# apache/horaedb

Hardware: NVIDIA H100
Metric: scanned rows/s (higher is better)
Workload: dtype f64

## Files before the change

horaedb_b200/csrc/fused_scan.cu:

```cuda
#include "fused_scan.h"

#include "block_scan.h"

#include <algorithm>
#include <chrono>
#include <cstdlib>

namespace horae {
namespace fused {

namespace {

constexpr int MAXC = 8;
constexpr int kWarpsPerCta = 8;

struct alignas(16) FRec {
  uint32_t item, local;
  uint64_t gkey;
  int64_t bucket;
  uint64_t count;
  double sum, mn, mx;
  uint64_t _pad;
};

struct VSeg { const uint8_t* base1; uint32_t n0, _pad; };

enum : uint32_t { K_RAW64 = 0, K_U32 = 1, K_I32 = 2, K_F32 = 3 };
inline uint32_t kind_of(uint32_t t) {
  return (t == T_U64 || t == T_I64 || t == T_F64) ? K_RAW64 : (t == T_F32 ? K_F32 : ((t == T_I8 || t == T_I16 || t == T_I32) ? K_I32 : K_U32));
}
constexpr uint64_t kI32KeyLo = (1ull << 63) - (1ull << 31), kI32KeyHi = (1ull << 63) + (1ull << 31) - 1;
constexpr int kHot = 4;

struct FParams {
  const SstDev* ssts;
  const RgSel* sel;
  const uint32_t* d_nsel;
  const uint8_t* const* bases;
  uint32_t split;
  uint32_t pcol[MAX_PREDS], pcls[MAX_PREDS];
  uint32_t pbloom[MAX_PREDS];
  uint64_t phash[MAX_PREDS];
  int nslots;
  uint32_t col[MAXC], kind[MAXC], cls[MAXC];
  int npk;
  int has_group, has_ts, value_slot, global_mode;
  int hot_slot[kHot];
  uint64_t hot_flip[kHot], hot_lo[kHot], hot_span[kHot];
  int hot_haspred[kHot];
  int npred;
  int pslot[MAX_PREDS];
  uint32_t pop[MAX_PREDS];
  uint64_t plit[MAX_PREDS];
  int64_t window_ms;
  const uint8_t* scratch;
  uint64_t scratch_stride;
  int region[MAXC];
  int value_stored;
  VSeg* vseg;
  FRec* rec;
  uint32_t rec_cap;
  uint32_t* item_cnt;
  unsigned int* work;
  unsigned long long* counters;
  int* err;
};

__device__ __forceinline__ uint64_t ld_bytes8(const uint8_t* p) {
  uintptr_t a = reinterpret_cast<uintptr_t>(p);
  uint32_t sh = uint32_t(a & 7) * 8;
  const uint64_t* q = reinterpret_cast<const uint64_t*>(a & ~uintptr_t(7));
  uint64_t lo = __ldg(q), hi = __ldg(q + 1);
  return (lo >> sh) | ((hi << 1) << (63 - sh));
}
__device__ __forceinline__ uint32_t ld32u(const uint8_t* p) { return uint32_t(ld_bytes8(p)); }

__device__ __forceinline__ uint64_t widen_kind(uint64_t raw, uint32_t kind) {
  uint32_t r = uint32_t(raw);
  uint64_t v = raw;
  v = kind == K_U32 ? uint64_t(r) : v;
  v = kind == K_I32 ? uint64_t(int64_t(int32_t(r))) : v;
  v = kind == K_F32 ? uint64_t(__double_as_longlong(double(__uint_as_float(r)))) : v;
  return v;
}
__device__ __forceinline__ uint64_t load_kind(const uint8_t* base, uint32_t kind, uint32_t row) {
  return widen_kind(ld_bytes8(base + size_t(row) * (kind == K_RAW64 ? 8u : 4u)), kind);
}

__device__ __forceinline__ uint32_t literal_header(const uint8_t* p, uint32_t* len) {
  const uint32_t t = __ldg(p);
  uint32_t l = t >> 2, hdr = 1;
  if (l >= 60) {
    const uint32_t nb = l - 59;
    l = 0;
    for (uint32_t i = 0; i < nb; i++) l |= uint32_t(__ldg(p + 1 + i)) << (8 * i);
    hdr = 1 + nb;
  }
  *len = l + 1;
  return hdr;
}

__device__ __forceinline__ const uint8_t* slot_base_chase(const FParams& P, uint32_t si, int s) {
  RgSel rs = P.sel[si];
  SstDev sst = P.ssts[rs.sst];
  ChunkDev cd = sst.chunks[size_t(rs.rg) * sst.ncols + P.col[s]];
  PageDev pg = sst.pages[cd.first_page];
  const uint8_t* body = sst.bytes + pg.payload_off;
  const bool is_value = P.value_stored && s == P.value_slot;
  if (cd.codec == 1) {
    if (is_value && cd.stored) {
      const uint8_t* p = body;
      while (__ldg(p) & 0x80) p++;
      p++;
      uint32_t len0 = 0, len1 = 0;
      const uint32_t h0 = literal_header(p, &len0);
      const uint8_t* lit0 = p + h0;
      const uint32_t prefix = cd.optional ? 4 + ld32u(lit0) : 0;
      const uint32_t w = P.kind[s] == K_RAW64 ? 8u : 4u;
      VSeg v;
      v.n0 = (len0 - prefix) / w;
      v._pad = 0;
      v.base1 = lit0 + prefix;
      if (lit0 + len0 < body + pg.comp_size) v.base1 = lit0 + len0 + literal_header(lit0 + len0, &len1);
      P.vseg[si] = v;
      return lit0 + prefix;
    }
    body = P.scratch + rs.scratch_off + uint64_t(P.region[s]) * P.scratch_stride;
  }
  if (cd.optional) {
    uint32_t lv = ld32u(body);
    if (lv > pg.uncomp_size) { lv = 0; atomicExch(P.err, 202); }
    body += 4 + lv;
  }
  if (is_value) { VSeg v; v.base1 = body; v.n0 = rs.num_rows; v._pad = 0; P.vseg[si] = v; }
  return body;
}
__device__ __forceinline__ const uint8_t* slot_base(const FParams& P, uint32_t si, int s) { return P.bases[size_t(si) * MAXC + s]; }
__device__ __noinline__ uint64_t fetch_val(const FParams& P, uint32_t si, int s, uint32_t row) {
  return load_kind(slot_base(P, si, s), P.kind[s], row);
}

struct Bucket { int64_t start, lo, hi; };
__device__ __noinline__ Bucket bucket_range(int64_t ts, int64_t w) {
  constexpr int64_t kMin = INT64_MIN, kMax = INT64_MAX;
  const int64_t r = w - 1;
  Bucket b;
  b.start = ts / w * w;
  if (b.start > 0) { b.lo = b.start; b.hi = b.start > kMax - r ? kMax : b.start + r; }
  else if (b.start < 0) { b.lo = b.start < kMin + r ? kMin : b.start - r; b.hi = b.start; }
  else { b.lo = -r; b.hi = r; }
  return b;
}

__device__ __noinline__ bool later_alive_dup(const FParams& P, uint32_t si, uint32_t row) {
  uint64_t pk[MAX_PK];
  for (int k = 0; k < P.npk; k++) pk[k] = fetch_val(P, si, k, row);
  uint32_t nrows = P.sel[si].num_rows;
  uint32_t r = row + 1;
  for (;;) {
    if (r >= nrows) {
      si++;
      if (si >= *P.d_nsel) return false;
      nrows = P.sel[si].num_rows;
      r = 0;
      if (nrows == 0) continue;
    }
    for (int k = 0; k < P.npk; k++)
      if (fetch_val(P, si, k, r) != pk[k]) return false;
    bool ok = true;
    for (int p = 0; p < P.npred && ok; p++) ok = op_holds(cmp_widened(fetch_val(P, si, P.pslot[p], r), P.plit[p], P.cls[P.pslot[p]]), P.pop[p]);
    if (ok) return true;
    r++;
  }
}

__device__ __forceinline__ uint64_t shfl64(uint64_t v, int src) {
  uint32_t lo = __shfl_sync(0xffffffffu, uint32_t(v), src);
  uint32_t hi = __shfl_sync(0xffffffffu, uint32_t(v >> 32), src);
  return (uint64_t(hi) << 32) | lo;
}
__device__ __forceinline__ double shfl_xor_d(double v, int m) {
  uint64_t b = uint64_t(__double_as_longlong(v));
  uint32_t lo = __shfl_xor_sync(0xffffffffu, uint32_t(b), m);
  uint32_t hi = __shfl_xor_sync(0xffffffffu, uint32_t(b >> 32), m);
  return __longlong_as_double((long long)((uint64_t(hi) << 32) | lo));
}

struct Acc {
  bool open;
  uint64_t g;
  int64_t bstart, blo, bhi;
  uint64_t cnt;
  double sum, mn, mx;
};

__device__ __noinline__ void emit(const FParams& P, const Acc& a, uint32_t item, uint32_t local, uint32_t* slots) {
  if (slots[0] == slots[1]) { slots[0] = atomicAdd(&P.work[1], 32u); slots[1] = slots[0] + 32u; }
  unsigned int slot = slots[0]++;
  if (slot < P.rec_cap) {
    FRec r;
    r.item = item; r.local = local; r.gkey = a.g; r.bucket = a.bstart; r.count = a.cnt; r.sum = a.sum; r.mn = a.mn; r.mx = a.mx; r._pad = 0;
    P.rec[slot] = r;
  } else atomicExch(P.err, 201);
}

struct FileDev {
  const RgCol* rgcol;
  const uint32_t* rg_rows;
  uint32_t rg_base, nrg, ncols, _pad;
  const uint8_t* bytes;
};

__global__ void __launch_bounds__(256) slot_bases_kernel(const __grid_constant__ FParams P, const uint8_t** __restrict__ bases, int only_slot) {
  const uint32_t idx = blockIdx.x * blockDim.x + threadIdx.x;
  const uint32_t si = idx / MAXC;
  const int s = int(idx % MAXC);
  if (si >= *P.d_nsel || s >= P.nslots || (only_slot >= 0 && s != only_slot)) return;
  bases[idx] = slot_base_chase(P, si, s);
}

template <bool W4>
__global__ void __launch_bounds__(256) gate_sel_kernel(const __grid_constant__ FParams P, RgSel* __restrict__ sel, int gate_slot, uint64_t flip,
                                                       uint64_t lo, uint64_t span, uint8_t* __restrict__ flags) {
  __shared__ uint32_t s_last;
  const uint32_t nsel = *P.d_nsel;
  for (uint32_t si = blockIdx.x; si < nsel; si += gridDim.x) {
    const uint8_t* base = P.bases[size_t(si) * MAXC + gate_slot];
    const uint32_t nrows = sel[si].num_rows;
    if (threadIdx.x == 0) s_last = 0;
    __syncthreads();
    uint32_t last = 0;
    const bool aligned = (reinterpret_cast<uintptr_t>(base) & 7) == 0;
    if (W4 && aligned) {
      const uint2* b2 = reinterpret_cast<const uint2*>(base);
      const uint32_t npair = nrows >> 1;
#pragma unroll 4
      for (uint32_t i = threadIdx.x; i < npair; i += 256) {
        const uint2 v = __ldg(b2 + i);
        if ((v.x ^ uint32_t(flip)) - uint32_t(lo) <= uint32_t(span)) last = 2 * i + 1;
        if ((v.y ^ uint32_t(flip)) - uint32_t(lo) <= uint32_t(span)) last = 2 * i + 2;
      }
      if ((nrows & 1) && threadIdx.x == 0 && (ld32u(base + size_t(nrows - 1) * 4) ^ uint32_t(flip)) - uint32_t(lo) <= uint32_t(span)) last = nrows;
    } else {
#pragma unroll 4
      for (uint32_t i = threadIdx.x; i < nrows; i += 256) {
        bool pass;
        if (W4) pass = (ld32u(base + size_t(i) * 4) ^ uint32_t(flip)) - uint32_t(lo) <= uint32_t(span);
        else pass = (ld_bytes8(base + size_t(i) * 8) ^ flip) - lo <= span;
        if (pass) last = i + 1;
      }
    }
    for (int d = 16; d > 0; d >>= 1) { const uint32_t o = __shfl_down_sync(0xffffffffu, last, d); last = o > last ? o : last; }
    if ((threadIdx.x & 31) == 0 && last) atomicMax(&s_last, last);
    __syncthreads();
    if (threadIdx.x == 0) {
      const uint32_t l = s_last;
      flags[si] = l ? 1 : 0;
      sel[si].out_row = l ? (l + 1 < nrows ? l + 1 : nrows) : 0;
    }
    __syncthreads();
  }
}

__global__ void __launch_bounds__(1024) compact_sel_kernel(const RgSel* __restrict__ in, const uint8_t* __restrict__ flags, uint32_t* d_nsel,
                                                           RgSel* __restrict__ out, uint32_t* __restrict__ lpt) {
  __shared__ uint32_t s_w[1024 / 32 + 1];
  __shared__ uint32_t s_bin[1024];
  __shared__ uint32_t s_max;
  const uint32_t n = *d_nsel;
  const uint32_t per = (n + 1023u) / 1024u;
  const uint32_t lo = threadIdx.x * per;
  const uint32_t hi = lo + per < n ? lo + per : n;
  uint32_t cnt = 0;
  for (uint32_t i = lo; i < hi; i++) cnt += flags[i] != 0;
  s_bin[threadIdx.x] = 0;
  if (threadIdx.x == 0) s_max = 0;
  uint32_t m;
  uint32_t pos = block_excl_scan<1024>(cnt, &m, s_w);
  uint32_t mx = 0;
  for (uint32_t i = lo; i < hi; i++)
    if (flags[i]) { out[pos++] = in[i]; mx = in[i].out_row > mx ? in[i].out_row : mx; }
  if (lpt) {
    if (mx) atomicMax(&s_max, mx);
    __syncthreads();
    int shift = 0;
    while ((s_max >> shift) > 1023u) shift++;
    const uint32_t per2 = (m + 1023u) / 1024u;
    const uint32_t lo2 = threadIdx.x * per2, hi2 = lo2 + per2 < m ? lo2 + per2 : m;
    for (uint32_t i = lo2; i < hi2; i++) atomicAdd(&s_bin[1023u - (out[i].out_row >> shift)], 1u);
    __syncthreads();
    uint32_t nbin;
    const uint32_t start = block_excl_scan<1024>(s_bin[threadIdx.x], &nbin, s_w);
    s_bin[threadIdx.x] = start;
    __syncthreads();
    for (uint32_t i = lo2; i < hi2; i++) lpt[atomicAdd(&s_bin[1023u - (out[i].out_row >> shift)], 1u)] = i;
  }
  __syncthreads();
  if (threadIdx.x == 0) *d_nsel = m;
}

__global__ void __launch_bounds__(256) prune_rgs_kernel(const __grid_constant__ FParams P, const FileDev* __restrict__ files, int nfiles,
                                                        uint32_t total_rgs, int prune, uint32_t* __restrict__ keep_rows) {
  const uint32_t idx = blockIdx.x * blockDim.x + threadIdx.x;
  if (idx >= total_rgs) return;
  uint32_t f = 0;
  while (f + 1 < uint32_t(nfiles) && idx >= files[f + 1].rg_base) f++;
  const FileDev fd = files[f];
  const uint32_t rg = idx - fd.rg_base;
  const uint32_t rows = fd.rg_rows[rg];
  uint32_t keep = rows > 0;
  if (keep && prune) {
    const RgCol* rc = fd.rgcol + size_t(rg) * fd.ncols;
    for (int p = 0; p < P.npred && keep; p++) {
      const RgCol c = rc[P.pcol[p]];
      if (c.null_all) { keep = 0; break; }
      if (c.has_minmax && !minmax_may_match(c.mn, c.mx, P.plit[p], P.pop[p], P.pcls[p])) keep = 0;
      else if ((prune & 2) && P.pbloom[p] && c.bloom_blocks && !bloom::may_contain(fd.bytes + c.bloom_off, c.bloom_blocks, P.phash[p])) keep = 0;
    }
  }
  keep_rows[idx] = keep ? rows : 0;
}

__global__ void __launch_bounds__(1024) select_rgs_kernel(const FileDev* __restrict__ files, int nfiles, uint32_t total_rgs,
                                                          const uint32_t* keep_rows, RgSel* __restrict__ sel, uint32_t* d_nsel,
                                                          unsigned long long* counters, uint32_t smem_words, uint64_t scratch_per_rg) {
  extern __shared__ uint32_t s_keep[];
  __shared__ uint32_t s_w[1024 / 32 + 1];
  if (smem_words) {
    for (uint32_t i = threadIdx.x; i < total_rgs; i += 1024) s_keep[i] = keep_rows[i];
    __syncthreads();
    keep_rows = s_keep;
  }
  const uint32_t per = (total_rgs + 1023u) / 1024u;
  const uint32_t lo = threadIdx.x * per;
  const uint32_t hi = lo + per < total_rgs ? lo + per : total_rgs;
  uint32_t cnt = 0;
  unsigned long long rows_sel = 0;
  for (uint32_t i = lo; i < hi; i++) { const uint32_t r = keep_rows[i]; cnt += r > 0; rows_sel += r; }
  uint32_t nsel;
  uint32_t pos = block_excl_scan<1024>(cnt, &nsel, s_w);
  if (cnt) {
// ... 143 lines not shown
                                        int64_t ts, double v, double* s_vals, uint32_t* slots, int lane) {
  const double kInf = __longlong_as_double(0x7ff0000000000000LL);
  const bool has_val = P.value_slot >= 0;
  bool ext = keep && acc.open && (!P.has_group || g == acc.g) && (!HAS_TS || (ts >= acc.blo && ts <= acc.bhi));
  if (__ballot_sync(0xffffffffu, ext) == keep_mask) {
    acc.cnt += __popc(keep_mask);
    if (has_val) {
      const bool num = keep && v == v;
      double mn = num ? v : kInf, mx = num ? v : -kInf;
#pragma unroll
      for (int m = 1; m < 32; m <<= 1) {
        const double a = shfl_xor_d(mn, m), b = shfl_xor_d(mx, m);
        const bool later = (lane & m) != 0;
        mn = (later ? a <= mn : a < mn) ? a : mn;
        mx = (later ? b >= mx : b > mx) ? b : mx;
      }
      acc.mn = mn < acc.mn ? mn : acc.mn;
      acc.mx = mx > acc.mx ? mx : acc.mx;
      acc.sum = seq_sum_slice(acc.sum, keep_mask, keep, v, s_vals, lane);
    }
    return;
  }
  uint64_t vb = uint64_t(__double_as_longlong(v));
  while (keep_mask) {
    int l = __ffs(keep_mask) - 1;
    keep_mask &= keep_mask - 1;
    uint64_t kg = P.has_group ? shfl64(g, l) : 0;
    int64_t kt = HAS_TS ? int64_t(shfl64(uint64_t(ts), l)) : 0;
    if (!acc.open || kg != acc.g || (HAS_TS && (kt < acc.blo || kt > acc.bhi))) {
      if (acc.open) { if (lane == 0) emit(P, acc, item, local, slots); local++; }
      acc.open = true; acc.g = kg; acc.cnt = 0; acc.sum = 0.0; acc.mn = kInf; acc.mx = -kInf;
      if (HAS_TS) { Bucket b = bucket_range(kt, P.window_ms); acc.bstart = b.start; acc.blo = b.lo; acc.bhi = b.hi; }
      else { acc.bstart = 0; acc.blo = 0; acc.bhi = 0; }
    }
    acc.cnt++;
    if (has_val) {
      double x = __longlong_as_double((long long)shfl64(vb, l));
      acc.sum += x;
      if (acc.cnt == 1 || x < acc.mn) acc.mn = x;
      if (acc.cnt == 1 || x > acc.mx) acc.mx = x;
    }
  }
}

__device__ __forceinline__ double to_double_kind(uint64_t raw, uint32_t kind, uint32_t cls) {
  uint64_t wv = widen_kind(raw, kind);
  return cls == C_FLOAT ? __longlong_as_double((long long)wv) : (cls == C_SIGNED ? double(int64_t(wv)) : double(wv));
}

__device__ __forceinline__ uint64_t ld8(const uint8_t* q, uint32_t sh, uint32_t i) {
  const uint64_t* p = reinterpret_cast<const uint64_t*>(q) + i;
  uint64_t lo = __ldg(p), hi = __ldg(p + 1);
  uint32_t w0 = uint32_t(lo), w1 = uint32_t(lo >> 32), w2 = uint32_t(hi), w3 = uint32_t(hi >> 32);
  const bool up = (sh & 32u) != 0;
  const uint32_t s = sh & 31u;
  uint32_t a = up ? w1 : w0, b = up ? w2 : w1, c = up ? w3 : w2;
  return (uint64_t(__funnelshift_r(b, c, s)) << 32) | __funnelshift_r(a, b, s);
}
__device__ __forceinline__ uint32_t ld4(const uint8_t* q, uint32_t sh, uint32_t i) {
  const uint32_t* p = reinterpret_cast<const uint32_t*>(q) + i;
  uint32_t lo = __ldg(p), hi = __ldg(p + 1);
  return __funnelshift_r(lo, hi, sh);
}

struct VCur {
  const uint8_t *q0, *q1;
  uint32_t s0, s1;
  uint32_t split;
};
__device__ __forceinline__ uint64_t ldv(const VCur& V, bool v8, uint32_t i) {
  const bool a = i < V.split;
  const uint8_t* q = a ? V.q0 : V.q1;
  const uint32_t sh = a ? V.s0 : V.s1;
  const uint32_t j = a ? i : i - V.split;
  return v8 ? ld8(q, sh, j) : uint64_t(ld4(q, sh, j));
}

template <int NH>
struct Hot {
  const uint8_t* q[NH];
  uint32_t sh[NH];
  uint64_t flip[NH], lo[NH], span[NH];
  bool haspred[NH];
};

template <int kU, int NH, int X, bool HAS_TS, bool dense>
__device__ __forceinline__ uint32_t process_block(const FParams& P, const Hot<NH>& H, const VCur& V, Acc& acc, uint32_t& local,
                                                  uint32_t& n_alive, uint32_t& n_keep, uint32_t& n_full, uint32_t item, uint32_t csi, uint32_t row,
                                                  uint32_t lim, uint32_t nrows, bool pf, double* s_vals, uint32_t* slots, int lane) {
  uint64_t hv[kU][NH];
  uint64_t vv[kU];
  uint64_t halo[2] = {0, 0};
  const uint32_t last = nrows - 1;
  if (pf) {
    const uint32_t prow = row + 2 * 32 * kU;
#pragma unroll
    for (int h = 0; h < NH; h++) {
      const bool w4 = h >= 2 && ((X >> (h - 2)) & 1);
      const uint32_t per_line = w4 ? 32u : 16u;
      const uint32_t r = prow + uint32_t(lane) * per_line;
      if (uint32_t(lane) <= (32u * kU) / per_line && r < nrows)
        asm volatile("prefetch.global.L2 [%0];" ::"l"(H.q[h] + size_t(r) * (w4 ? 4 : 8)));
    }
  }
  n_full += lim - row < 32u * kU ? lim - row : 32u * kU;
#pragma unroll
  for (int u = 0; u < kU; u++) {
    uint32_t i = row + u * 32 + lane;
    i = i < last ? i : last;
#pragma unroll
    for (int h = 0; h < NH; h++) {
      const bool w4 = h >= 2 && ((X >> (h - 2)) & 1);
      hv[u][h] = w4 ? uint64_t(ld4(H.q[h], H.sh[h], i)) : ld8(H.q[h], H.sh[h], i);
    }
  }
  const bool v8 = P.value_slot >= 0 && P.kind[P.value_slot] == K_RAW64;
  if (dense) {
    uint32_t i = row + kU * 32;
    i = i < last ? i : last;
    halo[0] = ld8(H.q[0], H.sh[0], i);
    halo[1] = ld8(H.q[1], H.sh[1], i);
#pragma unroll
    for (int u = 0; u < kU; u++) {
      uint32_t i2 = row + u * 32 + lane;
      i2 = i2 < last ? i2 : last;
      vv[u] = ldv(V, v8, i2);
    }
  }
  uint32_t kept_in_block = 0;
#pragma unroll
  for (int u = 0; u < kU; u++) {
    const uint32_t i = row + u * 32 + lane;
    bool alive = i < lim;
#pragma unroll
    for (int h = 0; h < NH; h++) {
      const bool w4 = h >= 2 && ((X >> (h - 2)) & 1);
      if (H.haspred[h]) {
        if (w4) alive = alive && ((uint32_t(hv[u][h]) ^ uint32_t(H.flip[h])) - uint32_t(H.lo[h]) <= uint32_t(H.span[h]));
        else alive = alive && ((hv[u][h] ^ H.flip[h]) - H.lo[h] <= H.span[h]);
      }
    }
    const unsigned alive_mask = __ballot_sync(0xffffffffu, alive);
    if (alive_mask == 0) continue;
    uint64_t n0 = shfl64(hv[u][0], (lane + 1) & 31), n1 = shfl64(hv[u][1], (lane + 1) & 31);
    if (u + 1 < kU) {
      uint64_t f0 = shfl64(hv[u + 1 < kU ? u + 1 : u][0], 0), f1 = shfl64(hv[u + 1 < kU ? u + 1 : u][1], 0);
      if (lane == 31) { n0 = f0; n1 = f1; }
    } else {
      if (!dense && (alive_mask >> 31)) {
        uint32_t ih = row + kU * 32;
        ih = ih < last ? ih : last;
        halo[0] = ld8(H.q[0], H.sh[0], ih);
        halo[1] = ld8(H.q[1], H.sh[1], ih);
      }
      if (lane == 31) { n0 = halo[0]; n1 = halo[1]; }
    }
    bool keep = alive;
    if (alive) {
      bool same = true;
      if (i + 1 < nrows) {
        same = n0 == hv[u][0] && n1 == hv[u][1];
        for (int k = 2; k < P.npk && same; k++) same = fetch_val(P, csi, k, i + 1) == fetch_val(P, csi, k, i);
      }
      if (same && (i + 1 < nrows || csi + 1 < *P.d_nsel)) keep = !later_alive_dup(P, csi, i);
    }
    const unsigned keep_mask = __ballot_sync(0xffffffffu, keep);
    n_alive += __popc(alive_mask);
    n_keep += __popc(keep_mask);
    kept_in_block += __popc(keep_mask);
    if (!P.global_mode && keep_mask) {
      double v = 0.0;
      if (P.value_slot >= 0) {
        uint64_t raw = vv[u];
        if (!dense) raw = keep ? ldv(V, v8, i) : 0ull;
        v = to_double_kind(raw, P.kind[P.value_slot], P.cls[P.value_slot]);
      }
      walk_slice<HAS_TS>(P, acc, local, item, keep_mask, keep, hv[u][0], int64_t(hv[u][1]), v, s_vals, slots, lane);
    }
  }
  return kept_in_block;
}

template <int kU, int NH, int X, int kGS>
__device__ __forceinline__ uint32_t gate_sweep(const Hot<NH>& H, uint32_t row, uint32_t lim, uint32_t nrows, int lane) {
  constexpr int G = NH - 1;
  constexpr bool w4 = G >= 2 && ((X >> (G - 2)) & 1);
  {
    constexpr uint32_t per_line = w4 ? 32u : 16u;
    const uint32_t r = row + 2u * 32u * kGS + uint32_t(lane) * per_line;
    if (uint32_t(lane) < (32u * kGS) / per_line + 1 && r < nrows)
      asm volatile("prefetch.global.L2 [%0];" ::"l"(H.q[G] + size_t(r) * (w4 ? 4 : 8)));
  }
  const uint32_t last = nrows - 1;
  uint64_t gv[kGS];
#pragma unroll
  for (int u = 0; u < kGS; u++) {
    uint32_t i = row + u * 32 + lane;
    i = i < last ? i : last;
    gv[u] = w4 ? uint64_t(ld4(H.q[G], H.sh[G], i)) : ld8(H.q[G], H.sh[G], i);
  }
  uint32_t bm = 0;
#pragma unroll
  for (int u = 0; u < kGS; u++) {
    bool pass = w4 ? ((uint32_t(gv[u]) ^ uint32_t(H.flip[G])) - uint32_t(H.lo[G]) <= uint32_t(H.span[G]))
                   : ((gv[u] ^ H.flip[G]) - H.lo[G] <= H.span[G]);
    pass = pass && (row + u * 32 + lane < lim);
    if (__ballot_sync(0xffffffffu, pass)) bm |= 1u << (u / kU);
  }
  return bm;
}

template <int kU, int NH, int X, int kGS>
__device__ __forceinline__ void prefetch_blocks(const Hot<NH>& H, const uint8_t* vq, bool has_val, bool v8, uint32_t bm, uint32_t row,
                                                uint32_t nrows, int lane) {
#pragma unroll
  for (int h = 0; h < NH - 1; h++) {
    const bool w4 = h >= 2 && ((X >> (h - 2)) & 1);
    const uint32_t off = uint32_t(lane) * (w4 ? 32u : 16u);
    uint32_t blk = off / (32u * kU);
    blk = blk < uint32_t(kGS / kU) ? blk : uint32_t(kGS / kU) - 1;
    if (off <= 32u * kGS && ((bm >> blk) & 1u) && row + off < nrows)
      asm volatile("prefetch.global.L2 [%0];" ::"l"(H.q[h] + size_t(row + off) * (w4 ? 4 : 8)));
  }
  if (has_val) {
    const uint32_t off = uint32_t(lane) * (v8 ? 16u : 32u);
    uint32_t blk = off / (32u * kU);
    blk = blk < uint32_t(kGS / kU) ? blk : uint32_t(kGS / kU) - 1;
    if (off <= 32u * kGS && ((bm >> blk) & 1u) && row + off < nrows)
      asm volatile("prefetch.global.L2 [%0];" ::"l"(vq + size_t(row + off) * (v8 ? 8 : 4)));
  }
}

template <int kU, int kMinBlocks, int NH, int X, bool HAS_TS, bool GATED>
__global__ void __launch_bounds__(kWarpsPerCta * 32, kMinBlocks) fused_scan_kernel(const __grid_constant__ FParams P,
                                                                                    const uint64_t* __restrict__ adj) {
  __shared__ double s_vals_all[kWarpsPerCta][32];
  __shared__ uint32_t s_slots[kWarpsPerCta][2];
  const int lane = threadIdx.x & 31, wid = threadIdx.x >> 5;
  double* s_vals = s_vals_all[wid];
  uint32_t* slots = s_slots[wid];
  if (lane == 0) { slots[0] = 0; slots[1] = 0; }
  __syncwarp();
  const uint32_t nsel = *P.d_nsel;
  const uint32_t nitems = nsel * P.split;
  constexpr int kGS = ((NH - 1) >= 2 && ((X >> (NH - 3)) & 1)) ? 16 : 8;
  const double kInf = __longlong_as_double(0x7ff0000000000000LL);
  Hot<NH> H;
#pragma unroll
  for (int h = 0; h < NH; h++) {
    H.flip[h] = P.hot_flip[h]; H.lo[h] = P.hot_lo[h]; H.span[h] = P.hot_span[h]; H.haspred[h] = P.hot_haspred[h] != 0;
    H.q[h] = nullptr; H.sh[h] = 0;
  }
  VCur V;
  V.q0 = nullptr; V.q1 = nullptr; V.s0 = 0; V.s1 = 0; V.split = 0xffffffffu;
  auto set_cursor = [&](uint32_t si) {
#pragma unroll
    for (int h = 0; h < NH; h++) {
      const uintptr_t a = reinterpret_cast<uintptr_t>(slot_base(P, si, P.hot_slot[h]));
      const bool w4 = h >= 2 && ((X >> (h - 2)) & 1);
      const uintptr_t m = w4 ? 3 : 7;
      H.q[h] = reinterpret_cast<const uint8_t*>(a & ~m);
      H.sh[h] = uint32_t(a & m) * 8;
    }
    if (P.value_slot >= 0) {
      const uintptr_t a = reinterpret_cast<uintptr_t>(slot_base(P, si, P.value_slot));
      const uintptr_t m = P.kind[P.value_slot] == K_RAW64 ? 7 : 3;
      V.q0 = reinterpret_cast<const uint8_t*>(a & ~m);
      V.s0 = uint32_t(a & m) * 8;
      if (P.value_stored) {
        const VSeg vg = P.vseg[si];
        const uintptr_t b = reinterpret_cast<uintptr_t>(vg.base1);
        V.q1 = reinterpret_cast<const uint8_t*>(b & ~m);
        V.s1 = uint32_t(b & m) * 8;
        V.split = vg.n0;
      }
    }
  };
  for (;;) {
    uint32_t item = 0;
    if (lane == 0) item = atomicAdd(&P.work[0], 1u);
    item = __shfl_sync(0xffffffffu, item, 0);
    if (item >= nitems) {
      if (lane == 0) for (uint32_t sl = slots[0]; sl < slots[1]; sl++) if (sl < P.rec_cap) P.rec[sl].item = 0xffffffffu;
      return;
    }
    const uint64_t beg = adj[item], end = adj[item + 1];
    uint32_t csi = uint32_t(beg >> 32), row = uint32_t(beg);
    const uint32_t esi = uint32_t(end >> 32), erow = uint32_t(end);
    uint32_t local = 0, n_alive = 0, n_keep = 0, n_full = 0;
    if (beg < end) {
      Acc acc;
      acc.open = false; acc.g = 0; acc.bstart = 0; acc.blo = 0; acc.bhi = 0; acc.cnt = 0; acc.sum = 0.0; acc.mn = kInf; acc.mx = -kInf;
      bool dense = false;
      uint32_t bm = 0, sweep_kept = 0;
      uint32_t nrows = P.sel[csi].num_rows;
      set_cursor(csi);
      for (;;) {
        if (row >= nrows) {
          csi++;
          row = 0;
          if (csi > esi || (csi == esi && erow == 0) || csi >= nsel) break;
          nrows = P.sel[csi].num_rows;
          set_cursor(csi);
        }
        const uint32_t lim = csi == esi ? erow : nrows;
        if (row >= lim) break;
        if (dense) {
          const uint32_t kept = process_block<kU, NH, X, HAS_TS, true>(P, H, V, acc, local, n_alive, n_keep, n_full, item, csi, row, lim, nrows,
                                                                      true, s_vals, slots, lane);
          dense = kept >= 32u * kU / 4;
          row += 32 * kU;
          continue;
        }
        uint32_t brow = row;
        if (GATED) {
          if (bm == 0) {
            bm = gate_sweep<kU, NH, X, kGS>(H, row, lim, nrows, lane);
            sweep_kept = 0;
            if (bm == 0) { row += 32u * kGS; continue; }
            prefetch_blocks<kU, NH, X, kGS>(H, V.q0, P.value_slot >= 0, P.value_slot >= 0 && P.kind[P.value_slot] == K_RAW64, bm, row, nrows, lane);
          }
          brow = row + (__ffs(bm) - 1) * 32u * kU;
          bm &= bm - 1;
        }
        const uint32_t kept = process_block<kU, NH, X, HAS_TS, false>(P, H, V, acc, local, n_alive, n_keep, n_full, item, csi, brow, lim, nrows,
                                                                     !GATED, s_vals, slots, lane);
        if (GATED) {
          sweep_kept += kept;
          if (bm == 0) {
            const uint32_t swept = lim - row < 32u * kGS ? lim - row : 32u * kGS;
            dense = P.value_slot >= 0 && sweep_kept >= swept / 4;
            row += 32u * kGS;
          }
        } else {
          dense = P.value_slot >= 0 && kept >= 32u * kU / 4;
          row += 32 * kU;
        }
      }
// ... 167 lines not shown
      if (nhot == kHot) return NOT_APPLICABLE;
      h = nhot++;
      hot_slot[h] = pslot[i];
    }
    uint64_t key = pred_literal(preds[i], t) ^ order_flip(t);
    switch (preds[i].op) {
      case HG_OP_EQ: klo[h] = std::max(klo[h], key); khi[h] = std::min(khi[h], key); break;
      case HG_OP_LT: if (key == 0) empty_interval = true; else khi[h] = std::min(khi[h], key - 1); break;
      case HG_OP_LE: khi[h] = std::min(khi[h], key); break;
      case HG_OP_GT: if (key == ~0ull) empty_interval = true; else klo[h] = std::max(klo[h], key + 1); break;
      default: klo[h] = std::max(klo[h], key); break;
    }
  }
  for (int h = 0; h < kHot; h++) if (klo[h] > khi[h]) empty_interval = true;
  for (int h = 2; h < nhot; h++) {
    const uint32_t t = schema->types[slots[hot_slot[h]]];
    if (type_width(t) == 8) continue;
    if (type_is_signed(t) ? (khi[h] < kI32KeyLo || klo[h] > kI32KeyHi) : klo[h] > 0xffffffffull) empty_interval = true;
  }
  if (nhot == 4 && type_width(schema->types[slots[hot_slot[2]]]) < type_width(schema->types[slots[hot_slot[3]]])) {
    std::swap(hot_slot[2], hot_slot[3]);
    std::swap(klo[2], klo[3]);
    std::swap(khi[2], khi[3]);
  }

  static const bool trace = getenv("HORAE_TRACE") != nullptr;
  auto now = [] { return std::chrono::steady_clock::now(); };
  auto us = [](std::chrono::steady_clock::time_point a, std::chrono::steady_clock::time_point b) { return std::chrono::duration<double, std::micro>(b - a).count(); };
  auto t0 = now();
  std::vector<SstResident*> files;
  uint64_t rows_in_files = 0;
  for (size_t i = 0; i < n; i++) {
    auto it = e->ssts.find(ssts[i].id);
    if (it == e->ssts.end()) return set_error(HG_ERR_INTERNAL, "sst not resident after load");
    SstResident* f = it->second.get();
    rows_in_files += f->rows_total;
    if (f->rows_total == 0) continue;
    for (uint32_t c : slots)
      if (!f->col_all_single[c] || !f->col_null_none[c] || f->col_any_zstd[c]) return NOT_APPLICABLE;
    if (!global_mode && (!f->col_has_minmax[0] || (has_ts && !f->col_has_minmax[1]))) return NOT_APPLICABLE;
    files.push_back(f);
  }
  if (files.size() > 1) {
    std::vector<Pk0Range> ranges;
    std::vector<size_t> order;
    for (SstResident* f : files) ranges.push_back(f->pk0);
    if (!pk0_disjoint(ranges, schema->types[0], &order)) return NOT_APPLICABLE;
    const std::vector<SstResident*> given = files;
    for (size_t j = 0; j < order.size(); j++) files[j] = given[order[j]];
  }
  uint32_t total_rgs = 0;
  for (SstResident* f : files) total_rgs += uint32_t(f->rg_rows.size());
  out->gtype = has_group ? schema->types[0] : uint32_t(T_U64);
  out->gwidth = has_group ? type_width(out->gtype) : 8;
  if (empty_interval) {
    for (DevBuf* b : {&out->gkey, &out->bucket, &out->count, &out->sum, &out->mn, &out->mx}) CU_TRY(b->alloc(16, e->stream));
    out->G = 0;
    e->stats.rows_in_files = rows_in_files;
    e->stats.path = 1;
    return HG_OK;
  }
  bool slot_snappy[MAXC] = {false};
  uint64_t slot_comp[MAXC] = {0};
  uint64_t scratch_stride = 0;
  bool value_stored = false, value_all_stored = true;
  for (size_t i = 0; i < slots.size(); i++)
    for (SstResident* f : files) {
      const uint32_t c = slots[i];
      if (f->col_any_snappy[c]) { slot_snappy[i] = true; scratch_stride = std::max<uint64_t>(scratch_stride, f->col_max_scratch[c]); }
      slot_comp[i] += f->col_comp_bytes[c];
      if (int(i) == value_slot) {
        if (f->col_snappy_any_stored[c]) value_stored = true;
        if (f->col_any_snappy[c] && !f->col_snappy_all_stored[c]) value_all_stored = false;
      }
    }
  if (value_slot >= 0) {
    if (!slot_snappy[value_slot]) value_stored = false;
    for (int h = 0; h < nhot; h++) if (hot_slot[h] == value_slot) value_stored = false;
    for (int k2 = 0; k2 < int(schema->num_primary_keys); k2++) if (k2 == value_slot) value_stored = false;
  }
  scratch_stride = (scratch_stride + 255) & ~uint64_t(255);
  int region[MAXC];
  int nregions = 0;
  for (size_t i = 0; i < slots.size(); i++) region[i] = (slot_snappy[i] && !(value_stored && value_all_stored && int(i) == value_slot)) ? nregions++ : -1;
  const bool need_snappy = nregions > 0;
  auto t1 = now();

  uint64_t bound = 1;
  if (!global_mode) {
    if (type_is_float(schema->types[0])) return NOT_APPLICABLE;
    bound = 0;
    if (!has_ts) {
      for (SstResident* f : files) bound += f->group_bound;
    } else {
      for (SstResident* f : files) {
        const size_t ncols = size_t(f->meta.ncols);
        for (size_t g = 0; g < f->rg_rows.size(); g++) {
          const RgCol* rc = &f->rgcol[g * ncols];
          const uint64_t rows = f->rg_rows[g];
          uint64_t span = rc[0].mx - rc[0].mn + 1;
          uint64_t per = std::min<uint64_t>((rc[1].mx - rc[1].mn) / uint64_t(agg->window_ms), 1ull << 33) + 2;
          uint64_t gcount = (span == 0 || span > (1ull << 32) || per > (1ull << 32)) ? rows : span * per;
          bound += std::min<uint64_t>(gcount, rows) + 1;
        }
      }
    }
    if (bound > rows_in_files / 32 + 1024) return NOT_APPLICABLE;
  }
  if (bound >= 0xfffffff0ull || rows_in_files >= 0xfffffff0ull) return NOT_APPLICABLE;

  cudaStream_t s = e->stream;
  Launch L = e->L();
  uint32_t split = 1;
  static const int items_per_warp = getenv("HORAE_ITEMS_PER_WARP") ? atoi(getenv("HORAE_ITEMS_PER_WARP")) : 4;
  while (split < 8 && uint64_t(total_rgs) * split < uint64_t(kNumSMs) * 32 * uint64_t(items_per_warp)) split *= 2;
  const uint32_t nitems = total_rgs * split;
  DevBuf d_ssts, d_files, d_sel, d_sel2, d_rec, d_item, d_work, d_adj, d_keep, d_bsum, d_bases, d_vseg, d_gflags, d_scratch, d_lpt;
  CU_TRY(d_work.alloc(256, s));
  CU_TRY(cudaMemsetAsync(d_work.p, 0, 256, s));
  uint8_t* const zblock = static_cast<uint8_t*>(d_work.p);
  unsigned long long* const counters_p = reinterpret_cast<unsigned long long*>(zblock + 64);
  int* const err_p = reinterpret_cast<int*>(zblock + 128);
  const uint64_t rec_cap = bound + uint64_t(kNumSMs) * 8 * kWarpsPerCta * 32;
  CU_TRY(d_rec.alloc(size_t(rec_cap) * sizeof(FRec) + 64, s));
  CU_TRY(d_item.alloc(size_t(nitems + 1) * sizeof(uint32_t) + 64, s));
  CU_TRY(d_adj.alloc(size_t(nitems + 2) * sizeof(uint64_t), s));
  CU_TRY(d_sel.alloc(size_t(total_rgs + 1) * sizeof(RgSel), s));
  CU_TRY(d_keep.alloc(size_t(total_rgs + 1) * sizeof(uint32_t), s));
  CU_TRY(d_bsum.alloc(1024 * sizeof(uint32_t), s));
  CU_TRY(d_bases.alloc(size_t(total_rgs + 1) * MAXC * sizeof(uint8_t*), s));
  if (value_stored) CU_TRY(d_vseg.alloc(size_t(total_rgs + 1) * sizeof(VSeg), s));
  if (need_snappy) {
    CU_TRY(d_sel2.alloc(size_t(total_rgs + 1) * sizeof(RgSel), s));
    CU_TRY(d_gflags.alloc(size_t(total_rgs) + 16, s));
    CU_TRY(d_lpt.alloc(size_t(total_rgs + 1) * sizeof(uint32_t), s));
    CU_TRY(d_scratch.alloc(size_t(total_rgs) * size_t(nregions) * scratch_stride + 256, s));
  }
  if ((uint64_t(nitems) + 1023) / 1024 > 1024) return NOT_APPLICABLE;
  CU_TRY(out->gkey.alloc(size_t(bound) * 8 + 16, s));
  CU_TRY(out->bucket.alloc(size_t(bound) * 8 + 16, s));
  CU_TRY(out->count.alloc(size_t(bound) * 8 + 16, s));
  CU_TRY(out->sum.alloc(size_t(bound) * 8 + 16, s));
  CU_TRY(out->mn.alloc(size_t(bound) * 8 + 16, s));
  CU_TRY(out->mx.alloc(size_t(bound) * 8 + 16, s));
  AggOut ao{out->gkey.p, out->bucket.as<int64_t>(), out->count.as<uint64_t>(), out->sum.as<double>(), out->mn.as<double>(), out->mx.as<double>()};

  auto t2 = now();
  unsigned long long hc[4] = {0, 0, 0, 0};
  int herr = 0;
  uint32_t hw[2] = {0, 0};
  if (total_rgs > 0) {
    std::vector<SstDev> sd(files.size());
    std::vector<FileDev> fdv(files.size());
    uint32_t rgb = 0;
    for (size_t i = 0; i < files.size(); i++) {
      SstResident* f = files[i];
      sd[i] = SstDev{f->d_bytes, f->d_pages, f->d_chunks, uint32_t(f->meta.ncols), uint32_t(f->meta.rgs.size())};
      fdv[i] = FileDev{f->d_rgcol, f->d_rg_rows, rgb, uint32_t(f->rg_rows.size()), uint32_t(f->meta.ncols), 0, f->d_bytes};
      rgb += uint32_t(f->rg_rows.size());
    }
    CU_TRY(d_ssts.alloc(sd.size() * sizeof(SstDev), s));
    CU_TRY(d_files.alloc(fdv.size() * sizeof(FileDev), s));
    size_t stage_off = 0;
    int urc = stage_upload(e, d_ssts.p, sd.data(), sd.size() * sizeof(SstDev), &stage_off);
    if (!urc) urc = stage_upload(e, d_files.p, fdv.data(), fdv.size() * sizeof(FileDev), &stage_off);
    if (urc) return urc;

    FParams P;
    std::memset(&P, 0, sizeof(P));
    P.ssts = d_ssts.as<SstDev>();
    P.sel = d_sel.as<RgSel>();
    P.d_nsel = d_work.as<uint32_t>() + 3;
    P.bases = d_bases.as<const uint8_t*>();
    P.split = split;
    P.nslots = int(slots.size());
    for (size_t i = 0; i < slots.size(); i++) {
      uint32_t t = schema->types[slots[i]];
      P.col[i] = slots[i];
      P.kind[i] = kind_of(t);
      P.cls[i] = cmp_class(t);
    }
    P.npk = int(schema->num_primary_keys);
    P.has_group = has_group;
    P.has_ts = has_ts;
    P.value_slot = value_slot;
    P.global_mode = global_mode;
    int xmask = 0;
    for (int h = 0; h < kHot; h++) {
      const int sl = h < nhot ? hot_slot[h] : 0;
      const uint32_t t = schema->types[slots[sl]];
      const bool w8 = (t == T_U64 || t == T_I64 || t == T_F64);
      P.hot_slot[h] = sl;
      P.hot_haspred[h] = (h < nhot && (klo[h] != 0 || khi[h] != ~0ull)) ? 1 : 0;
      uint64_t lo = klo[h], hi = khi[h];
      if (w8) P.hot_flip[h] = order_flip(t);
      else if (type_is_signed(t)) {
        P.hot_flip[h] = 1ull << 31;
        lo = lo < kI32KeyLo ? 0 : lo - kI32KeyLo;
        hi = hi > kI32KeyHi ? 0xffffffffull : hi - kI32KeyLo;
      } else {
        P.hot_flip[h] = 0;
        hi = std::min<uint64_t>(hi, 0xffffffffull);
      }
      P.hot_lo[h] = lo;
      P.hot_span[h] = hi >= lo ? hi - lo : 0;
      if (h >= 2 && h < nhot && !w8) xmask |= 1 << (h - 2);
    }
    P.npred = int(np);
    for (size_t i = 0; i < np; i++) {
      P.pslot[i] = pslot[i];
      P.pop[i] = preds[i].op;
      P.plit[i] = pred_literal(preds[i], schema->types[preds[i].column]);
      P.pcol[i] = preds[i].column;
      P.pcls[i] = cmp_class(schema->types[preds[i].column]);
      P.pbloom[i] = preds[i].op == HG_OP_EQ && bloom_literal_hash(P.plit[i], schema->types[preds[i].column], &P.phash[i]) ? 1u : 0u;
    }
    P.window_ms = has_ts ? agg->window_ms : 1;
    P.scratch = d_scratch.as<uint8_t>();
    P.scratch_stride = scratch_stride;
    for (int i = 0; i < MAXC; i++) P.region[i] = i < int(slots.size()) ? region[i] : -1;
    P.value_stored = value_stored ? 1 : 0;
    P.vseg = d_vseg.as<VSeg>();
    P.rec = d_rec.as<FRec>();
    P.rec_cap = uint32_t(rec_cap);
    P.item_cnt = d_item.as<uint32_t>();
    P.work = d_work.as<unsigned int>();
    P.counters = counters_p;
    P.err = err_p;

    int ctas = int(std::min<uint64_t>((uint64_t(nitems) + kWarpsPerCta - 1) / kWarpsPerCta, uint64_t(kNumSMs) * 8));
    static const bool env_nogate = getenv("HORAE_NO_GATE") != nullptr;
    const bool gated = !env_nogate && !(e->flags & HG_FLAG_NO_LATE_MATERIALIZATION) && P.hot_haspred[nhot - 1] != 0;
    prune_rgs_kernel<<<(total_rgs + 255) / 256, 256, 0, s>>>(P, d_files.as<FileDev>(), int(files.size()), total_rgs,
                                                             (e->flags & HG_FLAG_NO_PRUNING) ? 0 : ((e->flags & HG_FLAG_NO_BLOOM_FILTER) ? 1 : 3),
                                                             d_keep.as<uint32_t>());
    L.tick();
    {
      CU_TRY(cudaFuncSetAttribute(select_rgs_kernel, cudaFuncAttributeMaxDynamicSharedMemorySize, 200 * 1024));
      const uint32_t smem_words = size_t(total_rgs) * 4 <= 200 * 1024 ? total_rgs : 0;
      select_rgs_kernel<<<1, 1024, size_t(smem_words) * 4, s>>>(d_files.as<FileDev>(), int(files.size()), total_rgs, d_keep.as<uint32_t>(),
                                                                d_sel.as<RgSel>(), d_work.as<uint32_t>() + 3, counters_p, smem_words,
                                                                uint64_t(nregions) * scratch_stride);
    }
    L.tick();
    CU_TRY(cudaEventRecord(e->evd0, s));
    if (need_snappy) {
      auto make_job = [&](const std::vector<int>& job_slots, unsigned int* ticket) {
        k::SnappyJob J;
        std::memset(&J, 0, sizeof(J));
        J.ssts = P.ssts; J.sel = P.sel; J.d_nsel = P.d_nsel; J.nsel = 0; J.ncols = int(job_slots.size());
        std::vector<int> ord(job_slots.size());
        for (size_t i = 0; i < ord.size(); i++) ord[i] = int(i);
        std::stable_sort(ord.begin(), ord.end(), [&](int a, int b) { return slot_comp[job_slots[a]] > slot_comp[job_slots[b]]; });
        for (size_t i = 0; i < job_slots.size(); i++) {
          J.col[i] = slots[job_slots[i]];
          J.region[i] = uint32_t(region[job_slots[i]]);
          J.order[i] = uint8_t(ord[i]);
          J.skip_stored[i] = (value_stored && job_slots[i] == value_slot) ? 1 : 0;
        }
        J.fixed_stride = scratch_stride; J.scratch = d_scratch.as<uint8_t>(); J.ticket = ticket; J.err = err_p;
        return J;
      };
      unsigned int* tickets = reinterpret_cast<unsigned int*>(zblock + 136);
      const int gate_slot = hot_slot[nhot - 1];
      std::vector<int> first, rest;
      for (int i = 0; i < int(slots.size()); i++) {
        if (region[i] < 0) continue;
        if (gated && i == gate_slot) first.push_back(i); else rest.push_back(i);
      }
      if (!first.empty()) {
        k::snappy_pages(L, make_job(first, tickets), total_rgs);
        slot_bases_kernel<<<(total_rgs * MAXC + 255) / 256, 256, 0, s>>>(P, d_bases.as<const uint8_t*>(), gate_slot);
        L.tick();
        const uint32_t gt = schema->types[slots[gate_slot]];
        const bool w4 = !(gt == T_U64 || gt == T_I64 || gt == T_F64);
        if (w4) gate_sel_kernel<true><<<kNumSMs * 8, 256, 0, s>>>(P, d_sel.as<RgSel>(), gate_slot, P.hot_flip[nhot - 1], P.hot_lo[nhot - 1], P.hot_span[nhot - 1], d_gflags.as<uint8_t>());
        else gate_sel_kernel<false><<<kNumSMs * 8, 256, 0, s>>>(P, d_sel.as<RgSel>(), gate_slot, P.hot_flip[nhot - 1], P.hot_lo[nhot - 1], P.hot_span[nhot - 1], d_gflags.as<uint8_t>());
        L.tick();
        compact_sel_kernel<<<1, 1024, 0, s>>>(d_sel.as<RgSel>(), d_gflags.as<uint8_t>(), d_work.as<uint32_t>() + 3, d_sel2.as<RgSel>(), d_lpt.as<uint32_t>());
        L.tick();
        P.sel = d_sel2.as<RgSel>();
      }
      if (!rest.empty()) {
        k::SnappyJob J2 = make_job(rest, tickets + 1);
        if (!first.empty() && !has_ts)
          for (size_t i = 0; i < rest.size(); i++) J2.partial[i] = rest[i] != 0 ? 1 : 0;
        if (!first.empty()) { J2.sel = P.sel; J2.lpt = d_lpt.as<uint32_t>(); }
        k::snappy_pages(L, J2, total_rgs * uint32_t(rest.size()));
      }
    }
    CU_TRY(cudaEventRecord(e->evd1, s));
    slot_bases_kernel<<<(total_rgs * MAXC + 255) / 256, 256, 0, s>>>(P, d_bases.as<const uint8_t*>(), -1);
    L.tick();
    {
      const uint32_t nb = (nitems + 1 + kBoundsPerWarp - 1) / kBoundsPerWarp;
      const int bctas = int((uint64_t(nb) * 32 + 255) / 256);
      if (has_ts) item_bounds_kernel<true><<<bctas, 256, 0, s>>>(P, d_adj.as<uint64_t>());
      else item_bounds_kernel<false><<<bctas, 256, 0, s>>>(P, d_adj.as<uint64_t>());
      L.tick();
    }
    CU_TRY(cudaEventRecord(e->evk0, s));
    launch_fused<2, 4>(nhot, xmask, has_ts, gated, ctas, s, P, d_adj.as<uint64_t>());
    L.tick();
    CU_TRY(cudaEventRecord(e->evk1, s));
    if (global_mode) {
      global_count_kernel<<<1, 1, 0, s>>>(counters_p, ao);
      L.tick();
    } else {
      const uint32_t sblocks = (nitems + 1023) / 1024;
      item_scan_kernel<<<sblocks, 1024, 0, s>>>(d_item.as<uint32_t>(), d_work.as<uint32_t>() + 3, split, d_bsum.as<uint32_t>());
      L.tick();
      scatter_records_kernel<<<kNumSMs * 4, 256, 0, s>>>(d_rec.as<FRec>(), d_work.as<unsigned int>() + 1, d_item.as<uint32_t>(), d_bsum.as<uint32_t>(),
                                                     sblocks, d_work.as<uint32_t>() + 2, out->gwidth, ao, uint32_t(std::min<uint64_t>(bound, 0xffffffffu)), uint32_t(std::min<uint64_t>(rec_cap, 0xffffffffu)), err_p);
      L.tick();
    }
    auto t3 = now();
    {
      if (!e->h_small) CU_TRY(cudaMallocHost(&e->h_small, 256));
      uint8_t* const hb = static_cast<uint8_t*>(e->h_small);
      CU_TRY(cudaMemcpyAsync(hb, zblock, 192, cudaMemcpyDeviceToHost, s));
      CU_TRY(cudaStreamSynchronize(s));
      std::memcpy(hw, hb + 4, sizeof(hw));
      std::memcpy(hc, hb + 64, sizeof(hc));
      std::memcpy(&herr, hb + 128, sizeof(int));
    }
    auto t4 = now();
    if (trace) fprintf(stderr, "[fused] plan %.0f us, bound+alloc %.0f us, upload+launch %.0f us, wait %.0f us (row groups %u, max items %u)\n", us(t0, t1), us(t1, t2), us(t2, t3), us(t3, t4), total_rgs, nitems);
    if (herr >= 201 && herr <= 203) return set_error(HG_ERR_FORMAT, "fused scan: rows contradict their chunk statistics or a page is damaged (device error " + std::to_string(herr) + ")");
    if (herr) return set_error(HG_ERR_INTERNAL, "fused scan: device error " + std::to_string(herr));
    float kms = 0;
    cudaEventElapsedTime(&kms, e->evk0, e->evk1);
    e->stats.kernel_ms = kms;
    if (need_snappy) { cudaEventElapsedTime(&kms, e->evd0, e->evd1); e->stats.decomp_ms = kms; }
  }
  out->G = global_mode ? (hc[1] > 0 ? 1u : 0u) : hw[1];
  e->stats.rows_in_files = rows_in_files;
  e->stats.rows_decoded = hc[2];
  e->stats.rows_materialized = hc[3];
  e->stats.rows_filtered = hc[0];
  e->stats.rows_out = hc[1];
  e->stats.groups_out = out->G;
  e->stats.path = 1;
  return HG_OK;
}

}
}
```

Baseline: 51.01 billion.

## Precompute gate predicate bitmaps per row group and reuse them in fused sweep

New measurement: 52.59 billion (median of 6 runs). 3.1% higher.

```diff
diff --git a/horaedb_b200/csrc/fused_scan.cu b/horaedb_b200/csrc/fused_scan.cu
--- a/horaedb_b200/csrc/fused_scan.cu
+++ b/horaedb_b200/csrc/fused_scan.cu
@@ -57,6 +57,8 @@
   uint64_t scratch_stride;
   int region[MAXC];
   int value_stored;
+  int gate_bits;
+  uint64_t bits_off;
   VSeg* vseg;
   FRec* rec;
   uint32_t rec_cap;
@@ -211,52 +213,67 @@
   const uint8_t* bytes;
 };
 
-__global__ void __launch_bounds__(256) slot_bases_kernel(const __grid_constant__ FParams P, const uint8_t** __restrict__ bases, int only_slot) {
+__global__ void __launch_bounds__(256) slot_bases_kernel(const __grid_constant__ FParams P, const uint8_t** __restrict__ bases) {
   const uint32_t idx = blockIdx.x * blockDim.x + threadIdx.x;
   const uint32_t si = idx / MAXC;
   const int s = int(idx % MAXC);
-  if (si >= *P.d_nsel || s >= P.nslots || (only_slot >= 0 && s != only_slot)) return;
+  if (si >= *P.d_nsel || s >= P.nslots) return;
   bases[idx] = slot_base_chase(P, si, s);
 }
 
 template <bool W4>
-__global__ void __launch_bounds__(256) gate_sel_kernel(const __grid_constant__ FParams P, RgSel* __restrict__ sel, int gate_slot, uint64_t flip,
-                                                       uint64_t lo, uint64_t span, uint8_t* __restrict__ flags) {
+__global__ void __launch_bounds__(256, 8) gate_rg_kernel(const __grid_constant__ FParams P, RgSel* __restrict__ sel, int gate_slot, uint64_t flip,
+                                                      uint64_t lo, uint64_t span, uint8_t* __restrict__ flags) {
+  constexpr int kRows = W4 ? 8 : 4;
   __shared__ uint32_t s_last;
+  __shared__ const uint8_t* s_base[256];
   const uint32_t nsel = *P.d_nsel;
-  for (uint32_t si = blockIdx.x; si < nsel; si += gridDim.x) {
-    const uint8_t* base = P.bases[size_t(si) * MAXC + gate_slot];
-    const uint32_t nrows = sel[si].num_rows;
-    if (threadIdx.x == 0) s_last = 0;
-    __syncthreads();
-    uint32_t last = 0;
-    const bool aligned = (reinterpret_cast<uintptr_t>(base) & 7) == 0;
-    if (W4 && aligned) {
-      const uint2* b2 = reinterpret_cast<const uint2*>(base);
-      const uint32_t npair = nrows >> 1;
-#pragma unroll 4
-      for (uint32_t i = threadIdx.x; i < npair; i += 256) {
-        const uint2 v = __ldg(b2 + i);
-        if ((v.x ^ uint32_t(flip)) - uint32_t(lo) <= uint32_t(span)) last = 2 * i + 1;
-        if ((v.y ^ uint32_t(flip)) - uint32_t(lo) <= uint32_t(span)) last = 2 * i + 2;
-      }
-      if ((nrows & 1) && threadIdx.x == 0 && (ld32u(base + size_t(nrows - 1) * 4) ^ uint32_t(flip)) - uint32_t(lo) <= uint32_t(span)) last = nrows;
-    } else {
-#pragma unroll 4
-      for (uint32_t i = threadIdx.x; i < nrows; i += 256) {
-        bool pass;
-        if (W4) pass = (ld32u(base + size_t(i) * 4) ^ uint32_t(flip)) - uint32_t(lo) <= uint32_t(span);
-        else pass = (ld_bytes8(base + size_t(i) * 8) ^ flip) - lo <= span;
-        if (pass) last = i + 1;
-      }
-    }
-    for (int d = 16; d > 0; d >>= 1) { const uint32_t o = __shfl_down_sync(0xffffffffu, last, d); last = o > last ? o : last; }
-    if ((threadIdx.x & 31) == 0 && last) atomicMax(&s_last, last);
-    __syncthreads();
-    if (threadIdx.x == 0) {
-      const uint32_t l = s_last;
-      flags[si] = l ? 1 : 0;
-      sel[si].out_row = l ? (l + 1 < nrows ? l + 1 : nrows) : 0;
+  const int lane = threadIdx.x & 31;
+  for (uint32_t k0 = 0; blockIdx.x + k0 * gridDim.x < nsel; k0 += 256) {
+    {
+      const uint32_t si = blockIdx.x + (k0 + threadIdx.x) * gridDim.x;
+      if (si < nsel) s_base[threadIdx.x] = slot_base_chase(P, si, gate_slot);
+    }
+    for (uint32_t k = 0; k < 256; k++) {
+      const uint32_t si = blockIdx.x + (k0 + k) * gridDim.x;
+      if (si >= nsel) break;
+      if (threadIdx.x == 0) s_last = 0;
+      __syncthreads();
+      const uint8_t* base = s_base[k];
+      const RgSel rs = sel[si];
+      const uint32_t nrows = rs.num_rows;
+      uint32_t* bits = P.gate_bits ? reinterpret_cast<uint32_t*>(const_cast<uint8_t*>(P.scratch) + rs.scratch_off + P.bits_off) : nullptr;
+      const bool aligned = (reinterpret_cast<uintptr_t>(base) & (W4 ? 3 : 7)) == 0;
+      uint32_t last = 0;
+      const uint32_t nw = (nrows + 31) >> 5;
+      for (uint32_t i0 = 0; i0 < nw * 32; i0 += kRows * 256) {
+        uint64_t v[kRows];
+#pragma unroll
+        for (int u = 0; u < kRows; u++) {
+          const uint32_t i = i0 + u * 256 + threadIdx.x;
+          v[u] = 0;
+          if (i < nrows) {
+            if (W4) v[u] = aligned ? __ldg(reinterpret_cast<const uint32_t*>(base) + i) : ld32u(base + size_t(i) * 4);
+            else v[u] = aligned ? __ldg(reinterpret_cast<const unsigned long long*>(base) + i) : ld_bytes8(base + size_t(i) * 8);
+          }
+        }
+#pragma unroll
+        for (int u = 0; u < kRows; u++) {
+          const uint32_t i = i0 + u * 256 + threadIdx.x;
+          const bool pass = i < nrows && (W4 ? (uint32_t(v[u]) ^ uint32_t(flip)) - uint32_t(lo) <= uint32_t(span) : (v[u] ^ flip) - lo <= span);
+          if (pass) last = i + 1;
+          const uint32_t b = __ballot_sync(0xffffffffu, pass);
+          if (bits && lane == 0 && (i >> 5) < nw) bits[i >> 5] = b;
+        }
+      }
+      for (int d = 16; d > 0; d >>= 1) { const uint32_t o = __shfl_down_sync(0xffffffffu, last, d); last = o > last ? o : last; }
+      if (lane == 0 && last) atomicMax(&s_last, last);
+      __syncthreads();
+      if (threadIdx.x == 0) {
+        const uint32_t l = s_last;
+        flags[si] = l ? 1 : 0;
+        sel[si].out_row = l ? (l + 1 < nrows ? l + 1 : nrows) : 0;
+      }
     }
     __syncthreads();
   }
@@ -566,6 +583,7 @@
   uint32_t sh[NH];
   uint64_t flip[NH], lo[NH], span[NH];
   bool haspred[NH];
+  const uint32_t* gbits;
 };
 
 template <int kU, int NH, int X, bool HAS_TS, bool dense>
@@ -669,6 +687,24 @@
 __device__ __forceinline__ uint32_t gate_sweep(const Hot<NH>& H, uint32_t row, uint32_t lim, uint32_t nrows, int lane) {
   constexpr int G = NH - 1;
   constexpr bool w4 = G >= 2 && ((X >> (G - 2)) & 1);
+  if (H.gbits) {
+    const uint32_t* bw = H.gbits;
+    const uint32_t nw = (nrows + 31) >> 5;
+    uint32_t sb = 0;
+    const uint32_t r = row + uint32_t(lane) * 32u;
+    if (lane < kGS && r < lim) {
+      const uint32_t w = r >> 5;
+      const uint32_t a = __ldg(bw + w), b = w + 1 < nw ? __ldg(bw + w + 1) : 0u;
+      sb = __funnelshift_r(a, b, r & 31);
+      if (lim - r < 32) sb &= (1u << (lim - r)) - 1;
+    }
+    const unsigned m = __ballot_sync(0xffffffffu, sb != 0);
+    uint32_t bm = 0;
+#pragma unroll
+    for (int u = 0; u < kGS; u++)
+      if ((m >> u) & 1u) bm |= 1u << (u / kU);
+    return bm;
+  }
   {
     constexpr uint32_t per_line = w4 ? 32u : 16u;
     const uint32_t r = row + 2u * 32u * kGS + uint32_t(lane) * per_line;
@@ -737,7 +773,9 @@
   }
   VCur V;
   V.q0 = nullptr; V.q1 = nullptr; V.s0 = 0; V.s1 = 0; V.split = 0xffffffffu;
+  H.gbits = nullptr;
   auto set_cursor = [&](uint32_t si) {
+    if (GATED && P.gate_bits) H.gbits = reinterpret_cast<const uint32_t*>(P.scratch + P.sel[si].scratch_off + P.bits_off);
 #pragma unroll
     for (int h = 0; h < NH; h++) {
       const uintptr_t a = reinterpret_cast<uintptr_t>(slot_base(P, si, P.hot_slot[h]));
@@ -1071,8 +1109,13 @@
   scratch_stride = (scratch_stride + 255) & ~uint64_t(255);
   int region[MAXC];
   int nregions = 0;
+  uint32_t max_rg_rows = 0;
+  for (SstResident* f : files)
+    for (uint32_t r : f->rg_rows) max_rg_rows = std::max(max_rg_rows, r);
+  const uint64_t bits_bytes = (uint64_t((max_rg_rows + 31) / 32) * 4 + 255) & ~uint64_t(255);
   for (size_t i = 0; i < slots.size(); i++) region[i] = (slot_snappy[i] && !(value_stored && value_all_stored && int(i) == value_slot)) ? nregions++ : -1;
   const bool need_snappy = nregions > 0;
+  const uint64_t scratch_per_rg = uint64_t(nregions) * scratch_stride + bits_bytes;
   auto t1 = now();
 
   uint64_t bound = 1;
@@ -1123,7 +1166,7 @@
     CU_TRY(d_sel2.alloc(size_t(total_rgs + 1) * sizeof(RgSel), s));
     CU_TRY(d_gflags.alloc(size_t(total_rgs) + 16, s));
     CU_TRY(d_lpt.alloc(size_t(total_rgs + 1) * sizeof(uint32_t), s));
-    CU_TRY(d_scratch.alloc(size_t(total_rgs) * size_t(nregions) * scratch_stride + 256, s));
+    CU_TRY(d_scratch.alloc(size_t(total_rgs) * size_t(scratch_per_rg) + 256, s));
   }
   if ((uint64_t(nitems) + 1023) / 1024 > 1024) return NOT_APPLICABLE;
   CU_TRY(out->gkey.alloc(size_t(bound) * 8 + 16, s));
@@ -1220,6 +1263,10 @@
     int ctas = int(std::min<uint64_t>((uint64_t(nitems) + kWarpsPerCta - 1) / kWarpsPerCta, uint64_t(kNumSMs) * 8));
     static const bool env_nogate = getenv("HORAE_NO_GATE") != nullptr;
     const bool gated = !env_nogate && !(e->flags & HG_FLAG_NO_LATE_MATERIALIZATION) && P.hot_haspred[nhot - 1] != 0;
+    const int gate_slot = hot_slot[nhot - 1];
+    const bool gate_first = need_snappy && gated && region[gate_slot] >= 0;
+    P.gate_bits = gate_first ? 1 : 0;
+    P.bits_off = uint64_t(nregions) * scratch_stride;
     prune_rgs_kernel<<<(total_rgs + 255) / 256, 256, 0, s>>>(P, d_files.as<FileDev>(), int(files.size()), total_rgs,
                                                              (e->flags & HG_FLAG_NO_PRUNING) ? 0 : ((e->flags & HG_FLAG_NO_BLOOM_FILTER) ? 1 : 3),
                                                              d_keep.as<uint32_t>());
@@ -1229,7 +1276,7 @@
       const uint32_t smem_words = size_t(total_rgs) * 4 <= 200 * 1024 ? total_rgs : 0;
       select_rgs_kernel<<<1, 1024, size_t(smem_words) * 4, s>>>(d_files.as<FileDev>(), int(files.size()), total_rgs, d_keep.as<uint32_t>(),
                                                                 d_sel.as<RgSel>(), d_work.as<uint32_t>() + 3, counters_p, smem_words,
-                                                                uint64_t(nregions) * scratch_stride);
+                                                                scratch_per_rg);
     }
     L.tick();
     CU_TRY(cudaEventRecord(e->evd0, s));
@@ -1251,20 +1298,17 @@
         return J;
       };
       unsigned int* tickets = reinterpret_cast<unsigned int*>(zblock + 136);
-      const int gate_slot = hot_slot[nhot - 1];
       std::vector<int> first, rest;
       for (int i = 0; i < int(slots.size()); i++) {
         if (region[i] < 0) continue;
-        if (gated && i == gate_slot) first.push_back(i); else rest.push_back(i);
+        if (gate_first && i == gate_slot) first.push_back(i); else rest.push_back(i);
       }
       if (!first.empty()) {
         k::snappy_pages(L, make_job(first, tickets), total_rgs);
-        slot_bases_kernel<<<(total_rgs * MAXC + 255) / 256, 256, 0, s>>>(P, d_bases.as<const uint8_t*>(), gate_slot);
-        L.tick();
         const uint32_t gt = schema->types[slots[gate_slot]];
         const bool w4 = !(gt == T_U64 || gt == T_I64 || gt == T_F64);
-        if (w4) gate_sel_kernel<true><<<kNumSMs * 8, 256, 0, s>>>(P, d_sel.as<RgSel>(), gate_slot, P.hot_flip[nhot - 1], P.hot_lo[nhot - 1], P.hot_span[nhot - 1], d_gflags.as<uint8_t>());
-        else gate_sel_kernel<false><<<kNumSMs * 8, 256, 0, s>>>(P, d_sel.as<RgSel>(), gate_slot, P.hot_flip[nhot - 1], P.hot_lo[nhot - 1], P.hot_span[nhot - 1], d_gflags.as<uint8_t>());
+        if (w4) gate_rg_kernel<true><<<kNumSMs * 8, 256, 0, s>>>(P, d_sel.as<RgSel>(), gate_slot, P.hot_flip[nhot - 1], P.hot_lo[nhot - 1], P.hot_span[nhot - 1], d_gflags.as<uint8_t>());
+        else gate_rg_kernel<false><<<kNumSMs * 8, 256, 0, s>>>(P, d_sel.as<RgSel>(), gate_slot, P.hot_flip[nhot - 1], P.hot_lo[nhot - 1], P.hot_span[nhot - 1], d_gflags.as<uint8_t>());
         L.tick();
         compact_sel_kernel<<<1, 1024, 0, s>>>(d_sel.as<RgSel>(), d_gflags.as<uint8_t>(), d_work.as<uint32_t>() + 3, d_sel2.as<RgSel>(), d_lpt.as<uint32_t>());
         L.tick();
@@ -1279,7 +1323,7 @@
       }
     }
     CU_TRY(cudaEventRecord(e->evd1, s));
-    slot_bases_kernel<<<(total_rgs * MAXC + 255) / 256, 256, 0, s>>>(P, d_bases.as<const uint8_t*>(), -1);
+    slot_bases_kernel<<<(total_rgs * MAXC + 255) / 256, 256, 0, s>>>(P, d_bases.as<const uint8_t*>());
     L.tick();
     {
       const uint32_t nb = (nitems + 1 + kBoundsPerWarp - 1) / kBoundsPerWarp;
```
